# tomer-erez/Psychoacoustic-adverserial-attacks

Hardware: AMD Instinct MI355X
Metric: pgd_steps_per_sec (higher is better)
Workload: dtype bf16x3 (split-bf16 hi+lo, three MFMA passes, f32 accumulate: fp32-parity); 1 GPU; untargeted PGD, norm_type snr snr_db 40, Wav2Vec2-base (rule-generated weights), 32x10s 16 kHz clips per GPU, 150-token labels; global_batch=32, per_gpu_batch=32, samples_per_clip=160000, parallelism=dp1, hip_graph=True, hip_graph_replayed_steps=80

## Files before the change

### psychoacoustic-adverserial-attacks_amd/csrc/gemm.hip

```cpp
#include <algorithm>
#include <vector>

#include "gemm_dev.h"

namespace paa {

template <int ROWS, bool IS_A>
__device__ __forceinline__ void load_kc(const paa_gemm_desc& d, const float* __restrict__ base, int64_t ld, int r0,
                                        int k0, int rlim, float4 (&v)[ROWS / 32]) {
    const int tid = threadIdx.x;
    const int k = k0 + ((tid & 7) << 2);
    int64_t koff = k;
    int js = 0, kc = k;
    if (IS_A && d.a_kseg > 0) {
        js = k / d.a_kseg;
        kc = k - js * d.a_kseg;
        koff = (int64_t)js * d.a_kseg_stride + kc;
    }
#pragma unroll
    for (int i = 0; i < ROWS / 32; ++i) {
        const int r = r0 + (tid >> 3) + 32 * i;
        float4 x = make_float4(0.f, 0.f, 0.f, 0.f);
        bool ok = (r < rlim) && (k < d.K);
        const float* p;
        if (IS_A && d.a_window) {
            const int tr = r + js - d.a_pad;
            ok = ok && (tr >= 0) && (tr < d.a_rows_valid);
            p = base + (int64_t)tr * ld + kc;
        } else {
            p = base + (int64_t)r * ld + koff;
        }
        if (ok) {
// ... 518 lines not shown
    const int total = g.tiles_m * g.tiles_n * g.d.batch;
    const int blocks = resident > 0 ? std::min(total, resident) : total;
    hipLaunchKernelGGL((k_gemm_bf<BM, BN, PREC, WM, VEC, SEG, SWZ>), dim3(blocks), dim3(WM * 128), 0, st, g);
}

void launch_ring_cfg(int cfg, const GemmArgs& g, hipStream_t st);
void launch_ring2_cfg(int cfg, const GemmArgs& g, hipStream_t st);
int ring_tile_rows(int cfg);
int ring_tile_cols(int cfg);
bool ring_cfg_ok(int cfg, const paa_gemm_desc& d, bool forced = false);

static int g_ring_mode = 0;
struct GemmEnv { bool init = false, no_sq = false, no_r2 = false, kgroup = true, no_bil = false; };
static GemmEnv g_env;
static void gemm_env_refresh() {
#ifdef PAA_EXPERIMENTS
    auto on = [](const char* name, char v) { const char* e = getenv(name); return e && e[0] == v; };
    g_env.no_sq = on("PAA_NO_SQ", '1');
    g_env.no_r2 = on("PAA_NO_R2", '1');
    g_env.kgroup = !on("PAA_K_GROUP", '0');
    g_env.no_bil = on("PAA_NO_BIL", '1');
#endif
    g_env.init = true;
}
bool gemm_env_no_bil() {
    if (!g_env.init) gemm_env_refresh();
    return g_env.no_bil;
}
bool gemm_env_kgroup() {
    if (!g_env.init) gemm_env_refresh();
    return g_env.kgroup;
}

static int g_last_kind = EPK_GENERIC;
static int classify_epilogue(const paa_gemm_desc& d) {
#ifdef PAA_EXPERIMENTS
    { const char* e = getenv("PAA_NO_EPIK"); if (e && e[0] == '1') return EPK_GENERIC; }
#endif
    if (d.alpha != 1.f || d.accumulate || d.aux_bf16 || !d.precision) return EPK_GENERIC;
    const bool il = d.Cb_il && !d.Cb && !d.Cb_lo, planar = d.Cb && d.Cb_lo && !d.Cb_il, no_planes = !d.Cb && !d.Cb_lo && !d.Cb_il;
    const bool mask = d.row_period > 0;
    switch (d.act) {
        case PAA_ACT_GELU:
            return (d.C_pre && d.aux_gate && il && !d.C && !d.aux && !d.residual && !d.res_ln_stats) ? EPK_GELU_FWD : EPK_GENERIC;
        case PAA_ACT_GELU_GRAD:
            if (!(d.aux && d.aux_gate && (il || planar) && !d.bias && !d.C && !d.C_pre && !d.residual && !d.res_ln_stats && !mask)) return EPK_GENERIC;
#ifdef PAA_EXPERIMENTS
            { const char* e = getenv("PAA_EPIK_AHEAD"); if (e && e[0] == '2') return EPK_GELU_GRAD_LA2; if (e && e[0] == '4') return EPK_GELU_GRAD_LA4;
              if (e && e[0] == '1') return EPK_GELU_GRAD_LA1; }
#endif
            return EPK_GELU_GRAD;
        case PAA_ACT_NONE:
            if (d.C_pre || d.aux || d.aux_gate || mask) return EPK_GENERIC;
            if (d.C && no_planes && d.residual) {
                if (d.res_ln_stats) return d.bias ? EPK_RESID_LN : EPK_GENERIC;
                return d.bias ? EPK_GENERIC : EPK_RESID;
            }
            if (!d.C && planar && !d.residual && !d.res_ln_stats) return EPK_PLANES;
            return EPK_GENERIC;
        default: return EPK_GENERIC;
    }
}

template <int BN, int PREC>
static void launch_gemm(const GemmArgs& g, dim3 grid, hipStream_t st) {
    const bool akc = g.d.a_kcontig != 0, bkc = g.d.b_kcontig != 0;
    if (akc && bkc) hipLaunchKernelGGL((k_gemm<BN, PREC, true, true>), grid, dim3(G_NT), 0, st, g);
    else if (akc && !bkc) hipLaunchKernelGGL((k_gemm<BN, PREC, true, false>), grid, dim3(G_NT), 0, st, g);
    else if (!akc && bkc) hipLaunchKernelGGL((k_gemm<BN, PREC, false, true>), grid, dim3(G_NT), 0, st, g);
    else hipLaunchKernelGGL((k_gemm<BN, PREC, false, false>), grid, dim3(G_NT), 0, st, g);
}

struct GemmProf {
    bool on = false;
    std::vector<hipEvent_t> ev;
    std::vector<double> flops, bytes;
    std::vector<int> variant;
    size_t n = 0, cap = 0;
};
static GemmProf g_prof;

paa_status gemm(const paa_gemm_desc& d, hipStream_t st) {
    if ((!d.A && !d.A_il) || !d.B || (!d.C && !d.Cb && !d.Cb_il)) PAA_FAIL(PAA_ERR_ARG, "gemm: null operand");
    if (d.A_il) {
        if (!d.precision || !d.operand_bf16 || d.a_kseg > 0 || d.a_window || (d.lda & 31) || (d.K & 31) || (d.a_s1 & 31) || (d.a_s2 & 31) || ((uintptr_t)d.A_il & 15))
            PAA_FAIL(PAA_ERR_ARG, "gemm: A_il needs split precision, plain K-contiguous bf16 rows and lda / K / batch strides that are multiples of 32");
    }
    if (d.Cb_il) {
        if (!d.precision || d.Cb || d.Cb_lo || (d.ldc & 31) || (d.c_s1 & 31) || (d.c_s2 & 31) || ((uintptr_t)d.Cb_il & 15))
            PAA_FAIL(PAA_ERR_ARG, "gemm: Cb_il needs split precision, no Cb / Cb_lo, and ldc / batch strides that are multiples of 32");
    }
    if (d.accumulate && !d.C) PAA_FAIL(PAA_ERR_ARG, "gemm: accumulate needs the f32 result");
    if (d.Cb_lo && !d.Cb) PAA_FAIL(PAA_ERR_ARG, "gemm: Cb_lo without Cb");
    if (d.M <= 0 || d.N <= 0 || d.K <= 0 || d.batch <= 0 || d.batch2 <= 0) PAA_FAIL(PAA_ERR_SIZE, "gemm: bad dims %d %d %d", d.M, d.N, d.K);
    const int al = d.operand_bf16 ? 7 : 3;
    if ((d.lda & al) || (d.ldb & al) || (!d.A_il && ((uintptr_t)d.A & 15)) || ((uintptr_t)d.B & 15))
        PAA_FAIL(PAA_ERR_ARG, "gemm: operands must be 16-byte aligned with leading dimensions that are multiples of %d", al + 1);
    if ((d.a_s1 & al) || (d.a_s2 & al) || (d.b_s1 & al) || (d.b_s2 & al)) PAA_FAIL(PAA_ERR_ARG, "gemm: batch strides must be multiples of %d", al + 1);
    if (d.a_kseg > 0 && ((d.a_kseg & al) || (d.a_kseg_stride & al) || !d.a_kcontig)) PAA_FAIL(PAA_ERR_ARG, "gemm: bad K segmentation");
    if (d.operand_bf16) {
        if (!d.a_kcontig || !d.b_kcontig || (d.K & 7)) PAA_FAIL(PAA_ERR_ARG, "gemm: bf16 operands must be K-contiguous with K %% 8 == 0 (K=%d)", d.K);
        if (d.precision && ((!d.A_il && (!d.A_lo || ((uintptr_t)d.A_lo & 15))) || !d.B_lo || ((uintptr_t)d.B_lo & 15)))
            PAA_FAIL(PAA_ERR_ARG, "gemm: split precision needs aligned lo planes");
    }
    if (d.a_window && d.a_kseg <= 0) PAA_FAIL(PAA_ERR_ARG, "gemm: a_window needs a_kseg");
    if (d.act == PAA_ACT_GELU_GRAD && !d.aux) PAA_FAIL(PAA_ERR_ARG, "gemm: GELU_GRAD needs aux");
    if (d.res_ln_stats && (!d.residual || !d.res_ln_g || !d.res_ln_b || d.batch != 1 || d.act == PAA_ACT_GELU_GRAD ||
                           ((uintptr_t)d.res_ln_stats & 7) || ((uintptr_t)d.res_ln_g & 15) || ((uintptr_t)d.res_ln_b & 15)))
        PAA_FAIL(PAA_ERR_ARG, "gemm: res_ln_stats needs a residual, gain and bias (16-byte aligned), batch 1 and no GELU_GRAD");
    GemmArgs g;
    g.d = d;
    g.kind = EPK_GENERIC;
    const bool narrow = d.N <= 64;
    const int bn = narrow ? 64 : 128;
    auto al16 = [](const void* p) { return ((uintptr_t)p & 15) == 0; };
    const bool vec = d.operand_bf16 && !narrow && (d.N & 7) == 0 && (d.ldc & 7) == 0 && (d.c_s1 & 7) == 0 && (d.c_s2 & 7) == 0 &&
                     al16(d.C) && al16(d.C_pre) && al16(d.Cb) && al16(d.Cb_lo) && al16(d.Cb_il) &&
                     (!d.aux || (al16(d.aux) && (d.ld_aux & (d.aux_bf16 ? 7 : 3)) == 0 && (d.aux_s1 & 7) == 0 && (d.aux_s2 & 7) == 0)) &&
                     (!d.residual || (al16(d.residual) && (d.ld_res & 3) == 0 && (d.res_s1 & 3) == 0 && (d.res_s2 & 3) == 0)) &&
                     (!d.bias || (al16(d.bias) && (d.bias_s2 & 3) == 0)) &&
                     !(d.act == PAA_ACT_GELU_GRAD && d.residual) &&
                     63 * d.lda < (1ll << 30) && 63 * d.ldb < (1ll << 30) && (int64_t)d.M * d.ldc < (1ll << 30) && (int64_t)d.M * std::max(d.ld_aux, d.ld_res) < (1ll << 30);
    const bool tall = vec && d.a_kseg <= 0 && (d.K & 63) == 0 && d.M >= 2048;
    bool bm192 = false;
    if (tall && !d.precision) {
        static const int per_cu = std::max(1, blocks_per_cu(k_gemm_bf<256, 128, 0, 2, true, false>, 256));
        const int slots = per_cu * device_cus();
        const int64_t tn = cdiv(d.N, 128);
        const int64_t t256 = (int64_t)cdiv(d.M, 256) * tn * d.batch, t192 = (int64_t)cdiv(d.M, 192) * tn * d.batch;
        const double c256 = (double)((t256 + slots - 1) / slots) * 256.0, c192 = (double)((t192 + slots - 1) / slots) * 192.0 * 1.05;
        bm192 = c192 < c256;
    }
    int ring = 0;
    const bool forced2 = g_ring_mode >= 20 && vec && d.a_kseg <= 0 && ring_cfg_ok(g_ring_mode, d, true);
    if ((tall || forced2) && g_ring_mode != 1 && d.N >= 128) {
        const int64_t t256 = (int64_t)cdiv(d.M, 256) * cdiv(d.N, 256) * d.batch, t128 = (int64_t)cdiv(d.M, 256) * cdiv(d.N, 128) * d.batch;
        if (!g_env.init) gemm_env_refresh();
        const bool no_sq = g_env.no_sq;
        if (g_ring_mode >= 2) ring = g_ring_mode;
        else if (d.precision) {
            const int64_t slots = device_cus();
            const int64_t r256 = (t128 + slots - 1) / slots;
            const int64_t t192 = (int64_t)cdiv(d.M, 192) * cdiv(d.N, 128) * d.batch;
            const int64_t r192 = (t192 + 2 * slots - 1) / (2 * slots);
            const int64_t rsq = (t256 + slots - 1) / slots;
// ... 61 lines not shown
        const size_t lds = 2 * (size_t)npl * ((size_t)(128 * mi + taps - 1) * (d.a_kseg + 8) + 64 * (size_t)(4 * d.a_kseg + 8));
        if (lds <= 150 * 1024) {
            dim3 wgrid(cdiv(d.M, 128 * mi), d.batch);
#define PAA_WIN(P, KS_, MI_, WV_)                                                                                            \
            {                                                                                                                \
                static bool attr = false;                                                                                    \
                if (!attr) { PAA_HIP(hipFuncSetAttribute(reinterpret_cast<const void*>(&k_gemm_win<P, KS_, MI_, WV_>), hipFuncAttributeMaxDynamicSharedMemorySize, 152 * 1024)); attr = true; } \
                hipLaunchKernelGGL((k_gemm_win<P, KS_, MI_, WV_>), wgrid, dim3(WV_ * 64), lds, st, g, taps);                 \
            }
            if (prof) { g_prof.variant[g_prof.n] = 40 + (d.precision ? 4 : 0); }
            if (d.a_kseg == 48) {
                if (mi == 2) { if (d.precision) PAA_WIN(1, 48, 1, 8) else PAA_WIN(0, 48, 2, 4) }
                else { if (d.precision) PAA_WIN(1, 48, 1, 4) else PAA_WIN(0, 48, 1, 4) }
            }
            else { if (d.precision) PAA_WIN(1, 64, 1, 4) else PAA_WIN(0, 64, 1, 4) }
#undef PAA_WIN
            if (prof) { (void)hipEventRecord(g_prof.ev[2 * g_prof.n + 1], st); ++g_prof.n; }
            PAA_LAUNCH_CHECK();
            return PAA_OK;
        }
    }
    if (ring) {
        if (prof) g_prof.variant[g_prof.n] = (ring_bm == 192 ? (ring_bn == 128 ? 60 : 52) : (ring_bn == 256 ? 56 : 48)) + (d.precision ? 1 : 0);
#ifdef PAA_EXPERIMENTS
        if (ring == 13) launch_bf<192, 128, 1, 2, true, false, true>(g, st);
        else
#endif
        if (ring >= 20) {
            g.kind = g_last_kind = classify_epilogue(d);
            int taken = EPK_SHIPPED;
#ifdef PAA_EXPERIMENTS
            { const char* e = getenv("PAA_EPIK_MASK"); const int mask = e ? atoi(e) : 0; if (mask > 0) taken = mask; }
#endif
            if (!((taken >> g.kind) & 1)) g.kind = EPK_GENERIC;
            launch_ring2_cfg(ring, g, st);
        }
        else launch_ring_cfg(ring, g, st);
    } else if (d.operand_bf16) {
        const bool seg = d.a_kseg > 0 || (d.K & 63);
        if (narrow) {
            if (seg) { if (d.precision) launch_bf<128, 64, 1, 2, false, true>(g, st); else launch_bf<128, 64, 0, 2, false, true>(g, st); }
            else { if (d.precision) launch_bf<128, 64, 1, 2, false, false>(g, st); else launch_bf<128, 64, 0, 2, false, false>(g, st); }
        }
        else if (seg && vec && !d.precision) launch_bf<128, 128, 0, 2, true, true>(g, st);
        else if (seg) { if (d.precision) launch_bf<128, 128, 1, 2, false, true>(g, st); else launch_bf<128, 128, 0, 2, false, true>(g, st); }
        else if (tall) {
            if (d.precision) launch_bf<256, 128, 1, 4, true, false>(g, st);
            else if (bm192) launch_bf<192, 128, 0, 2, true, false>(g, st);
            else launch_bf<256, 128, 0, 2, true, false>(g, st);
        }
        else if (vec) { if (d.precision) launch_bf<128, 128, 1, 2, true, false>(g, st); else launch_bf<128, 128, 0, 2, true, false>(g, st); }
        else { if (d.precision) launch_bf<128, 128, 1, 2, false, false>(g, st); else launch_bf<128, 128, 0, 2, false, false>(g, st); }
    } else if (narrow) { if (d.precision) launch_gemm<64, 1>(g, grid, st); else launch_gemm<64, 0>(g, grid, st); }
    else { if (d.precision) launch_gemm<128, 1>(g, grid, st); else launch_gemm<128, 0>(g, grid, st); }
    if (prof) { (void)hipEventRecord(g_prof.ev[2 * g_prof.n + 1], st); ++g_prof.n; }
    PAA_LAUNCH_CHECK();
    return PAA_OK;
}

}

extern "C" paa_status paa_prof_enable(int max_launches) {
    using namespace paa;
    for (hipEvent_t e : g_prof.ev) (void)hipEventDestroy(e);
    g_prof.ev.clear(); g_prof.n = 0; g_prof.cap = 0; g_prof.on = false;
    if (max_launches <= 0) return PAA_OK;
    g_prof.ev.resize(2 * (size_t)max_launches);
    for (auto& e : g_prof.ev) PAA_HIP(hipEventCreate(&e));
    g_prof.flops.assign(max_launches, 0.0);
    g_prof.bytes.assign(max_launches, 0.0);
    g_prof.variant.assign(max_launches, 0);
    g_prof.cap = max_launches; g_prof.on = true;
    return PAA_OK;
}

extern "C" paa_status paa_prof_read(double* out256) {
    using namespace paa;
    if (!out256) PAA_FAIL(PAA_ERR_ARG, "paa_prof_read: null");
    for (int i = 0; i < 256; ++i) out256[i] = 0.0;
    if (g_prof.n == 0) return PAA_OK;
    PAA_HIP(hipEventSynchronize(g_prof.ev[2 * g_prof.n - 1]));
    for (size_t i = 0; i < g_prof.n; ++i) {
        float ms = 0.f;
        PAA_HIP(hipEventElapsedTime(&ms, g_prof.ev[2 * i], g_prof.ev[2 * i + 1]));
        const int v = g_prof.variant[i];
        out256[4 * v] += 1.0; out256[4 * v + 1] += ms; out256[4 * v + 2] += g_prof.flops[i]; out256[4 * v + 3] += g_prof.bytes[i];
    }
    g_prof.n = 0;
    return PAA_OK;
}

extern "C" paa_status paa_prof_pause(int paused) {
    paa::g_prof.on = !paused && paa::g_prof.cap > 0;
    return PAA_OK;
}

#ifdef PAA_EXPERIMENTS
extern "C" int paa_debug_last_epilogue_kind() { return paa::g_last_kind; }
#endif

extern "C" void paa_gemm_config(int ring_mode) { paa::g_ring_mode = ring_mode; paa::gemm_env_refresh(); }

extern "C" paa_status paa_gemm(const struct paa_gemm_desc* d, void* stream) {
    if (!d) { paa::set_error("paa_gemm: null descriptor"); return PAA_ERR_ARG; }
    return paa::gemm(*d, (hipStream_t)stream);
}
```

### psychoacoustic-adverserial-attacks_amd/csrc/gemm_dev.h

```cpp
#pragma once
#include "gemm.h"
#include "paa_common.h"

namespace paa {

typedef short bf16x8 __attribute__((ext_vector_type(8)));
typedef float f32x16 __attribute__((ext_vector_type(16)));

constexpr int G_BM = 128, G_BK = 32, G_LD = 40 , G_NT = 256;


struct GemmArgs {
    paa_gemm_desc d;
    int tiles_m, tiles_n;
    int kind;
};

enum { EPK_GENERIC = 0, EPK_GELU_FWD = 1, EPK_GELU_GRAD = 2, EPK_RESID = 3, EPK_RESID_LN = 4, EPK_PLANES = 5,
       EPK_GELU_GRAD_LA2 = 6, EPK_GELU_GRAD_LA4 = 7, EPK_GELU_GRAD_LA1 = 8, EPK_COUNT = 9 };
constexpr int EPK_SHIPPED = (1 << EPK_GELU_FWD) | (1 << EPK_GELU_GRAD) | (1 << EPK_PLANES);
enum { EPI_NO = 0, EPI_YES = 1, EPI_RT = 2 };
template <int S>
__device__ __forceinline__ bool epi_on(bool rt) {
    if constexpr (S == EPI_RT) return rt;
    else return S == EPI_YES;
}
struct EpiGeneric {
    static constexpr int ACT = -1, BIAS = EPI_RT, C = EPI_RT, CPRE = EPI_RT, X16 = EPI_RT, GATE = EPI_RT, CIL = EPI_RT, CB = EPI_RT, CBLO = EPI_RT,
                         RES = EPI_RT, RLN = EPI_RT, PERIOD = EPI_RT, ACCUM = EPI_RT;
    static constexpr bool ALPHA1 = false;
    static constexpr int AHEAD = 1;
    static constexpr bool SETTLE_EARLY = false;
};
struct EpiGeluFwd {
    static constexpr int ACT = PAA_ACT_GELU, BIAS = EPI_RT, C = EPI_NO, CPRE = EPI_YES, X16 = EPI_NO, GATE = EPI_YES, CIL = EPI_YES, CB = EPI_NO, CBLO = EPI_NO,
                         RES = EPI_NO, RLN = EPI_NO, PERIOD = EPI_RT, ACCUM = EPI_NO;
    static constexpr bool ALPHA1 = true;
    static constexpr int AHEAD = 1;
    static constexpr bool SETTLE_EARLY = false;
};
struct EpiGeluGrad {
    static constexpr int ACT = PAA_ACT_GELU_GRAD, BIAS = EPI_NO, C = EPI_NO, CPRE = EPI_NO, X16 = EPI_NO, GATE = EPI_YES, CIL = EPI_RT, CB = EPI_YES, CBLO = EPI_YES,
                         RES = EPI_NO, RLN = EPI_NO, PERIOD = EPI_NO, ACCUM = EPI_NO;
    static constexpr bool ALPHA1 = true;
    static constexpr int AHEAD = 1;
    static constexpr bool SETTLE_EARLY = true;
};
template <int AH>
struct EpiGeluGradAhead : EpiGeluGrad {
    static constexpr int AHEAD = AH;
    static constexpr bool SETTLE_EARLY = false;
};
struct EpiResid {
    static constexpr int ACT = PAA_ACT_NONE, BIAS = EPI_NO, C = EPI_YES, CPRE = EPI_NO, X16 = EPI_NO, GATE = EPI_NO, CIL = EPI_NO, CB = EPI_NO, CBLO = EPI_NO,
                         RES = EPI_YES, RLN = EPI_NO, PERIOD = EPI_NO, ACCUM = EPI_NO;
    static constexpr bool ALPHA1 = true;
    static constexpr int AHEAD = 1;
    static constexpr bool SETTLE_EARLY = false;
};
struct EpiResidLn {
    static constexpr int ACT = PAA_ACT_NONE, BIAS = EPI_YES, C = EPI_YES, CPRE = EPI_NO, X16 = EPI_NO, GATE = EPI_NO, CIL = EPI_NO, CB = EPI_NO, CBLO = EPI_NO,
                         RES = EPI_YES, RLN = EPI_YES, PERIOD = EPI_NO, ACCUM = EPI_NO;
    static constexpr bool ALPHA1 = true;
    static constexpr int AHEAD = 1;
    static constexpr bool SETTLE_EARLY = false;
};
struct EpiPlanes {
    static constexpr int ACT = PAA_ACT_NONE, BIAS = EPI_RT, C = EPI_NO, CPRE = EPI_NO, X16 = EPI_NO, GATE = EPI_NO, CIL = EPI_NO, CB = EPI_YES, CBLO = EPI_YES,
                         RES = EPI_NO, RLN = EPI_NO, PERIOD = EPI_NO, ACCUM = EPI_NO;
    static constexpr bool ALPHA1 = true;
    static constexpr int AHEAD = 1;
    static constexpr bool SETTLE_EARLY = false;
};

template <typename K>
inline int blocks_per_cu(K kernel, int threads) {
    int per = 0;
    if (hipOccupancyMaxActiveBlocksPerMultiprocessor(&per, kernel, threads, 0) != hipSuccess) return 0;
    return per;
}

template <int NJ, int MI>
__device__ __forceinline__ void epilogue(const paa_gemm_desc& d, f32x16 (&acc)[MI][NJ], int mw, int nw, int z1, int z2) {
    const int64_t coff = z1 * d.c_s1 + z2 * d.c_s2 + (int64_t)mw * d.ldc + nw;
    float* __restrict__ C = d.C ? d.C + coff : nullptr;
    const bool x16 = d.aux_bf16 != 0;
    float* __restrict__ Cp = (d.C_pre && !x16) ? d.C_pre + coff : nullptr;
    unsigned short* __restrict__ Cp16 = (d.C_pre && x16) ? reinterpret_cast<unsigned short*>(d.C_pre) + coff : nullptr;
    unsigned short* __restrict__ Cb = d.Cb ? reinterpret_cast<unsigned short*>(d.Cb) + coff : nullptr;
    unsigned short* __restrict__ Cbl = d.Cb_lo ? reinterpret_cast<unsigned short*>(d.Cb_lo) + coff : nullptr;
    unsigned short* __restrict__ Cil = d.Cb_il ? reinterpret_cast<unsigned short*>(d.Cb_il) + 2 * (z1 * d.c_s1 + z2 * d.c_s2) : nullptr;
    const int64_t xoff = z1 * d.aux_s1 + z2 * d.aux_s2 + (int64_t)mw * d.ld_aux + nw;
    const float* __restrict__ aux = (d.aux && !x16) ? d.aux + xoff : nullptr;
    const unsigned short* __restrict__ aux16 = (d.aux && x16) ? reinterpret_cast<const unsigned short*>(d.aux) + xoff : nullptr;
    const float* __restrict__ res = d.residual ? d.residual + z1 * d.res_s1 + z2 * d.res_s2 + (int64_t)mw * d.ld_res + nw : nullptr;
    const float* __restrict__ bias = d.bias ? d.bias + z2 * d.bias_s2 + nw : nullptr;
    const int ldc = (int)d.ldc, ld_aux = (int)d.ld_aux, ld_res = (int)d.ld_res;
    const int period = d.row_period;
    const int mrem0 = period > 0 ? mw % period : 0;
    const int act = d.act;
    const float alpha = d.alpha;
#pragma unroll
    for (int i = 0; i < MI; ++i) {
        const int64_t ro = (int64_t)(i * 32) * ldc;
        float* __restrict__ Ci = C ? C + ro : nullptr;
// ... 57 lines not shown
                }
                if (Cil) {
                    const int n = nw + dn;
                    const int64_t o = (int64_t)(mw + i * 32 + dm) * (2 * d.ldc) + ((n >> 5) << 6) + (n & 31);
                    const unsigned short h = bf16_bits(v);
                    Cil[o] = h;
                    Cil[o + 32] = bf16_bits(v - bf16_to_f32(h));
                }
            }
        }
    }
}

__device__ __forceinline__ float dpp_quad_xor1(float v) {
    return __int_as_float(__builtin_amdgcn_mov_dpp(__float_as_int(v), 0xB1, 0xF, 0xF, true));
}
__device__ __forceinline__ float dpp_quad_xor2(float v) {
    return __int_as_float(__builtin_amdgcn_mov_dpp(__float_as_int(v), 0x4E, 0xF, 0xF, true));
}
__device__ __forceinline__ void quad_transpose(float& x0, float& x1, float& x2, float& x3, bool o1, bool o2) {
    float s = dpp_quad_xor1(o1 ? x0 : x1);
    float t = dpp_quad_xor1(o1 ? x2 : x3);
    if (o1) { x0 = s; x2 = t; } else { x1 = s; x3 = t; }
    s = dpp_quad_xor2(o2 ? x0 : x2);
    t = dpp_quad_xor2(o2 ? x1 : x3);
    if (o2) { x0 = s; x1 = t; } else { x2 = s; x3 = t; }
}

__device__ __forceinline__ float mul_unfused(float a, float b) {
#pragma clang fp contract(off)
    return a * b;
}

__device__ __forceinline__ void epi_landed(const uint4& v) { asm volatile("" ::"v"(v.x), "v"(v.y), "v"(v.z), "v"(v.w)); }
template <int N>
__device__ __forceinline__ void epi_landed(const float (&v)[N]) {
#pragma unroll
    for (int k = 0; k < N; ++k) asm volatile("" ::"v"(v[k]));
}

template <int MI, bool FAST, typename T = EpiGeneric>
__device__ __forceinline__ void epilogue_vec(const paa_gemm_desc& d, f32x16 (&acc)[MI][2], int m0w, int n0w, int z1, int z2, int lane) {
    const int lr = lane & 31, lh = lane >> 5, qa = lr >> 2, qb = lr & 3;
    const bool o1 = qb & 1, o2 = qb & 2;
    const int col = n0w + 8 * qa;
    const int row0 = m0w + 4 * lh + qb;
    const bool col_ok = col < d.N;
    const int act = T::ACT < 0 ? d.act : T::ACT;
    const bool gg = act == PAA_ACT_GELU_GRAD;
    const int64_t cbase = z1 * d.c_s1 + z2 * d.c_s2;
    float* __restrict__ C = epi_on<T::C>(d.C != nullptr) ? d.C + cbase : nullptr;
    const bool has_c = T::C == EPI_RT ? C != nullptr : T::C == EPI_YES;
    const bool x16 = epi_on<T::X16>(d.aux_bf16 != 0);
    const bool gate = epi_on<T::GATE>(d.aux_gate != 0);
    float* __restrict__ Cp = (epi_on<T::CPRE>(d.C_pre != nullptr) && !x16) ? d.C_pre + cbase : nullptr;
    unsigned short* __restrict__ Cp16 = (epi_on<T::CPRE>(d.C_pre != nullptr) && x16) ? reinterpret_cast<unsigned short*>(d.C_pre) + cbase : nullptr;
    constexpr bool PRE_RT = T::CPRE == EPI_RT || T::X16 == EPI_RT;
    const bool has_cp = PRE_RT ? Cp != nullptr : (T::CPRE == EPI_YES && T::X16 == EPI_NO);
    const bool has_cp16 = PRE_RT ? Cp16 != nullptr : (T::CPRE == EPI_YES && T::X16 == EPI_YES);
    unsigned short* __restrict__ Cb = epi_on<T::CB>(d.Cb != nullptr) ? reinterpret_cast<unsigned short*>(d.Cb) + cbase : nullptr;
    unsigned short* __restrict__ Cbl = epi_on<T::CBLO>(d.Cb_lo != nullptr) ? reinterpret_cast<unsigned short*>(d.Cb_lo) + cbase : nullptr;
    const bool cil = epi_on<T::CIL>(d.Cb_il != nullptr);
    if (cil) { Cb = reinterpret_cast<unsigned short*>(d.Cb_il) + 2 * cbase; Cbl = Cb + 32; }
    const bool has_cb = (T::CIL == EPI_YES || T::CB == EPI_YES) ? true : (T::CIL == EPI_NO && T::CB == EPI_NO) ? false : Cb != nullptr;
    const bool has_cbl = (T::CIL == EPI_YES || T::CBLO == EPI_YES) ? true : (T::CIL == EPI_NO && T::CBLO == EPI_NO) ? false : Cbl != nullptr;
    const bool ex16 = gg && x16;
    const float* __restrict__ ex = gg ? (ex16 ? nullptr : d.aux + z1 * d.aux_s1 + z2 * d.aux_s2)
                                      : (epi_on<T::RES>(d.residual != nullptr) ? d.residual + z1 * d.res_s1 + z2 * d.res_s2 : nullptr);
    const unsigned short* __restrict__ exh = ex16 ? reinterpret_cast<const unsigned short*>(d.aux) + z1 * d.aux_s1 + z2 * d.aux_s2 : nullptr;
    constexpr bool EX_RT = T::ACT < 0 || T::X16 == EPI_RT || T::RES == EPI_RT;
    const bool has_ex = EX_RT ? ex != nullptr : (gg ? !ex16 : T::RES == EPI_YES);
    const bool has_exh = EX_RT ? exh != nullptr : ex16;
    const unsigned ldc = (unsigned)d.ldc, ldx = (unsigned)(gg ? d.ld_aux : d.ld_res);
    const unsigned co = (unsigned)row0 * ldc + (unsigned)col;
    const unsigned cob = cil ? (unsigned)row0 * 2u * ldc + (((unsigned)col >> 5) << 6) + ((unsigned)col & 31u) : co;
    const unsigned ldcb = cil ? 2u * ldc : ldc;
    float bv[8];
#pragma unroll
    for (int k = 0; k < 8; ++k) bv[k] = 0.f;
    if (epi_on<T::BIAS>(d.bias != nullptr) && col_ok) {
        const float* bp = d.bias + z2 * d.bias_s2;
        const float4 b0 = *reinterpret_cast<const float4*>(bp + (unsigned)col);
        const float4 b1 = *reinterpret_cast<const float4*>(bp + (unsigned)col + 4u);
        bv[0] = b0.x; bv[1] = b0.y; bv[2] = b0.z; bv[3] = b0.w; bv[4] = b1.x; bv[5] = b1.y; bv[6] = b1.z; bv[7] = b1.w;
    }
    const bool rln = epi_on<T::RLN>(d.res_ln_stats != nullptr) && !gg && has_ex;
    constexpr bool RLN_HELD = MI < 4;
    float lg[8], lb[8];
#pragma unroll
    for (int k = 0; k < 8; ++k) { lg[k] = 1.f; lb[k] = 0.f; }
    if (RLN_HELD && rln && col_ok) {
        const float4 g0 = *reinterpret_cast<const float4*>(d.res_ln_g + (unsigned)col), g1 = *reinterpret_cast<const float4*>(d.res_ln_g + (unsigned)col + 4u);
        const float4 b0 = *reinterpret_cast<const float4*>(d.res_ln_b + (unsigned)col), b1 = *reinterpret_cast<const float4*>(d.res_ln_b + (unsigned)col + 4u);
        lg[0] = g0.x; lg[1] = g0.y; lg[2] = g0.z; lg[3] = g0.w; lg[4] = g1.x; lg[5] = g1.y; lg[6] = g1.z; lg[7] = g1.w;
        lb[0] = b0.x; lb[1] = b0.y; lb[2] = b0.z; lb[3] = b0.w; lb[4] = b1.x; lb[5] = b1.y; lb[6] = b1.z; lb[7] = b1.w;
    }
    const int period = T::PERIOD == EPI_NO ? 0 : d.row_period;
    const int mrem0 = period > 0 ? row0 % period : 0;
    const float alpha = T::ALPHA1 ? 1.f : d.alpha;
    const bool accum = epi_on<T::ACCUM>(d.accumulate != 0);
    constexpr int NG = 4 * MI;
    constexpr int AH = T::AHEAD < NG ? T::AHEAD : NG - 1, NX = AH + 1;
    uint4 xv[NX][2];
    constexpr bool RS_AHEAD = T::RLN == EPI_YES;
    float rsv[NX][2];
    constexpr bool EARLY = T::SETTLE_EARLY && AH == 1 && T::ACT == PAA_ACT_GELU_GRAD && T::X16 != EPI_RT && T::C == EPI_NO && T::CPRE == EPI_NO;
    constexpr bool EX_ANY = EX_RT || T::ACT == PAA_ACT_GELU_GRAD || T::RES == EPI_YES;
#pragma unroll
    for (int u = 0; u < NX; ++u) { xv[u][0] = make_uint4(0u, 0u, 0u, 0u); xv[u][1] = xv[u][0]; rsv[u][0] = 0.f; rsv[u][1] = 1.f; }
    auto fetch = [&](int grp, uint4 (&v2)[2], float (&r2)[2]) {
        const unsigned rowc = (unsigned)min(row0 + (grp >> 2) * 32 + (grp & 3) * 8, d.M - 1);
        if (RS_AHEAD && rln) {
            const float2 st = *reinterpret_cast<const float2*>(d.res_ln_stats + 2 * (size_t)rowc);
            r2[0] = st.x; r2[1] = st.y;
        }
        const unsigned o = rowc * ldx + (col_ok ? (unsigned)col : 0u);
        if (has_ex) {
            v2[0] = *reinterpret_cast<const uint4*>(ex + o);
            v2[1] = *reinterpret_cast<const uint4*>(ex + o + 4u);
        } else if (has_exh) {
            v2[0] = *reinterpret_cast<const uint4*>(exh + o);
        }
    };
#pragma unroll
    for (int a = 0; a < AH; ++a) fetch(a, xv[a], rsv[a]);
#pragma unroll
    for (int grp = 0; grp < NG; ++grp) {
        const int i = grp >> 2, gq = grp & 3, u = grp % NX;
        if (grp + AH < NG) fetch(grp + AH, xv[(grp + AH) % NX], rsv[(grp + AH) % NX]);
        if (grp == 0) {
            if constexpr (T::BIAS != EPI_NO) epi_landed(bv);
            if constexpr (RLN_HELD && T::RLN != EPI_NO) { epi_landed(lg); epi_landed(lb); }
        }
        if constexpr (EX_ANY) { epi_landed(xv[u][0]); epi_landed(xv[u][1]); }
        if constexpr (RS_AHEAD) epi_landed(rsv[u]);
        const int dm = i * 32 + gq * 8;
        const bool live = col_ok && row0 + dm < d.M;
        bool dead = false;
        if (period > 0) {
            int rem = mrem0 + dm;
            if (rem >= period) rem = (period >= 256) ? rem - period : rem % period;
            dead = rem >= d.row_valid;
        }
        const unsigned ci = co + (unsigned)dm * ldc;
        float2 rst = make_float2(rsv[u][0], rsv[u][1]);
        if (!RS_AHEAD && rln && live) rst = *reinterpret_cast<const float2*>(d.res_ln_stats + 2 * (size_t)(row0 + dm));
        unsigned hp[4], lp[4], pp[4];
#pragma unroll
        for (int j = 0; j < 2; ++j) {
            float x[4] = {acc[i][j][4 * gq], acc[i][j][4 * gq + 1], acc[i][j][4 * gq + 2], acc[i][j][4 * gq + 3]};
            quad_transpose(x[0], x[1], x[2], x[3], o1, o2);
            float e4[4];
            if (ex16) {
                const unsigned w0 = j ? xv[u][0].z : xv[u][0].x, w1 = j ? xv[u][0].w : xv[u][0].y;
                e4[0] = __uint_as_float(w0 << 16); e4[1] = __uint_as_float(w0 & 0xFFFF0000u);
                e4[2] = __uint_as_float(w1 << 16); e4[3] = __uint_as_float(w1 & 0xFFFF0000u);
            } else {
                e4[0] = __uint_as_float(xv[u][j].x); e4[1] = __uint_as_float(xv[u][j].y);
                e4[2] = __uint_as_float(xv[u][j].z); e4[3] = __uint_as_float(xv[u][j].w);
            }
            if (rln) {
                if constexpr (RLN_HELD) {
#pragma unroll
                    for (int k = 0; k < 4; ++k) e4[k] = (e4[k] - rst.x) * rst.y * lg[4 * j + k] + lb[4 * j + k];
                } else {
                    float4 g4 = make_float4(1.f, 1.f, 1.f, 1.f), b4 = make_float4(0.f, 0.f, 0.f, 0.f);
                    if (col_ok) {
                        g4 = *reinterpret_cast<const float4*>(d.res_ln_g + (unsigned)col + 4u * j);
                        b4 = *reinterpret_cast<const float4*>(d.res_ln_b + (unsigned)col + 4u * j);
                    }
                    e4[0] = (e4[0] - rst.x) * rst.y * g4.x + b4.x; e4[1] = (e4[1] - rst.x) * rst.y * g4.y + b4.y;
                    e4[2] = (e4[2] - rst.x) * rst.y * g4.z + b4.z; e4[3] = (e4[3] - rst.x) * rst.y * g4.w + b4.w;
                }
            }
#pragma unroll
            for (int k = 0; k < 4; ++k) x[k] = x[k] * alpha + bv[4 * j + k];
            if (act == PAA_ACT_GELU) {
                float kp[4];
                if (FAST) {
#pragma unroll
                    for (int k = 0; k < 4; k += 2) {
                        f32x2 dg;
                        const f32x2 gv = gelu_both_fast2(f32x2{x[k], x[k + 1]}, dg);
                        kp[k] = gate ? dg.x : x[k]; kp[k + 1] = gate ? dg.y : x[k + 1];
                        x[k] = gv.x; x[k + 1] = gv.y;
                    }
                } else {
#pragma unroll
                    for (int k = 0; k < 4; ++k) {
                        kp[k] = gate ? gelu_grad_f(x[k]) : x[k];
                        x[k] = gelu_f(x[k]);
                    }
                }
                if (has_cp && live) *reinterpret_cast<float4*>(Cp + ci + 4u * j) = dead ? make_float4(0.f, 0.f, 0.f, 0.f) : make_float4(kp[0], kp[1], kp[2], kp[3]);
                if (has_cp16) {
                    pp[2 * j] = dead ? 0u : bf16_pack2(kp[0], kp[1]);
                    pp[2 * j + 1] = dead ? 0u : bf16_pack2(kp[2], kp[3]);
                }
                if (has_ex) {
#pragma unroll
                    for (int k = 0; k < 4; ++k) x[k] += e4[k];
                }
            } else if (gg) {
#pragma unroll
                for (int k = 0; k < 4; ++k) x[k] = mul_unfused(x[k], gate ? e4[k] : (FAST ? gelu_grad_fast(e4[k]) : gelu_grad_f(e4[k])));
            } else if (has_ex) {
#pragma unroll
                for (int k = 0; k < 4; ++k) x[k] += e4[k];
            }
            if (dead) {
#pragma unroll
                for (int k = 0; k < 4; ++k) x[k] = 0.f;
            }
            if (has_c && live) {
                if (accum) {
                    const float4 c0 = *reinterpret_cast<const float4*>(C + ci + 4u * j);
                    x[0] += c0.x; x[1] += c0.y; x[2] += c0.z; x[3] += c0.w;
                }
                *reinterpret_cast<float4*>(C + ci + 4u * j) = make_float4(x[0], x[1], x[2], x[3]);
            }
            if (has_cb) {
                const unsigned h01 = bf16_pack2(x[0], x[1]), h23 = bf16_pack2(x[2], x[3]);
                hp[2 * j] = h01; hp[2 * j + 1] = h23;
                if (has_cbl) {
                    lp[2 * j] = bf16_pack2(x[0] - __uint_as_float(h01 << 16), x[1] - __uint_as_float(h01 & 0xFFFF0000u));
                    lp[2 * j + 1] = bf16_pack2(x[2] - __uint_as_float(h23 << 16), x[3] - __uint_as_float(h23 & 0xFFFF0000u));
                }
            }
            __builtin_amdgcn_sched_barrier(0);
        }
        if constexpr (EARLY) {
            if (grp + 1 < NG) { epi_landed(xv[(grp + 1) % NX][0]); epi_landed(xv[(grp + 1) % NX][1]); }
        }
        if (has_cp16 && live && act == PAA_ACT_GELU) *reinterpret_cast<uint4*>(Cp16 + ci) = make_uint4(pp[0], pp[1], pp[2], pp[3]);
        if (has_cb && live) {
            const unsigned cb = cob + (unsigned)dm * ldcb;
            *reinterpret_cast<uint4*>(Cb + cb) = make_uint4(hp[0], hp[1], hp[2], hp[3]);
            if (has_cbl) *reinterpret_cast<uint4*>(Cbl + cb) = make_uint4(lp[0], lp[1], lp[2], lp[3]);
        }
    }
}

}
```

### psychoacoustic-adverserial-attacks_amd/csrc/gemm_ring2.hip

```cpp
#include <stdlib.h>

#include <algorithm>

#include "gemm_dev.h"

namespace paa {

bool gemm_env_no_bil();

namespace {

#if defined(PAA_R2_DEFER) && !defined(PAA_EXPERIMENTS)
#error "PAA_R2_DEFER is a diagnostic build: add -DPAA_EXPERIMENTS"
#endif
#ifndef PAA_R2_DEFER
#define PAA_R2_DEFER 1
#endif
#if (defined(PAA_R2_A_AUX) || defined(PAA_R2_B_AUX)) && !defined(PAA_EXPERIMENTS)
#error "PAA_R2_A_AUX / PAA_R2_B_AUX are diagnostic builds: add -DPAA_EXPERIMENTS"
#endif
#ifndef PAA_R2_A_AUX
#define PAA_R2_A_AUX 0
#endif
#ifndef PAA_R2_PRIO_BALANCE
// ... 311 lines not shown
                            for (int j = 0; j < NJ; ++j) { bh[j] = bhn[j]; bl[j] = bln[j]; }
                        }
                    }
                }
            if (!DEFER || last) {
                if (ahead) wait_vmcnt2<GA>(); else wait_vmcnt2<0>();
                __builtin_amdgcn_sched_barrier(0);
                __builtin_amdgcn_s_barrier();
                __builtin_amdgcn_sched_barrier(0);
            }
        }
#ifdef PAA_R2_STAMP
        const long long st_t1 = R2_NOW();
#endif
        epilogue_vec<MI, true, EPI>(d, acc, cur.m0 + wr * (BM / WR), cur.n0 + wc * (BN / WC), cur.z1, cur.z2, lane);
#ifdef PAA_R2_STAMP
        if (blockIdx.x == 0 && lane == 0 && st_tile < 16) {
            long long* o = g_r2_stamp + (wave * 16 + st_tile) * 6;
            o[0] = nk; o[1] = st_t1 - st_t0; o[2] = st_vm; o[3] = st_bar; o[4] = R2_NOW() - st_t1; o[5] = st_t0;
        }
        ++st_tile;
#endif
    }
}

template <int BM, int BN, int BK, int PREC, int WR, int WC, bool BIL, bool AIL, typename EPI = EpiGeneric>
void launch_ring2_il(const GemmArgs& g, hipStream_t st) {
    static const int per_cu = blocks_per_cu(k_gemm_ring2<BM, BN, BK, PREC, WR, WC, BIL, AIL, EPI>, WR * WC * 64);
    const int resident = per_cu * device_cus();
    const int total = g.tiles_m * g.tiles_n * g.d.batch;
    const int blocks = resident > 0 ? std::min(total, resident) : total;
    hipLaunchKernelGGL((k_gemm_ring2<BM, BN, BK, PREC, WR, WC, BIL, AIL, EPI>), dim3(blocks), dim3(WR * WC * 64), 0, st, g);
}
template <int BM, int BN, int BK, int WR, int WC, bool AIL>
void launch_ring2_kind(const GemmArgs& g, hipStream_t st) {
    switch (g.kind) {
        case EPK_GELU_FWD: launch_ring2_il<BM, BN, BK, 1, WR, WC, true, AIL, EpiGeluFwd>(g, st); return;
        case EPK_GELU_GRAD: launch_ring2_il<BM, BN, BK, 1, WR, WC, true, AIL, EpiGeluGrad>(g, st); return;
#ifdef PAA_EXPERIMENTS
        case EPK_GELU_GRAD_LA2: launch_ring2_il<BM, BN, BK, 1, WR, WC, true, AIL, EpiGeluGradAhead<2>>(g, st); return;
        case EPK_GELU_GRAD_LA4: launch_ring2_il<BM, BN, BK, 1, WR, WC, true, AIL, EpiGeluGradAhead<4>>(g, st); return;
        case EPK_GELU_GRAD_LA1: launch_ring2_il<BM, BN, BK, 1, WR, WC, true, AIL, EpiGeluGradAhead<1>>(g, st); return;
#endif
        default: break;
    }
    if constexpr (BM == 192) {
        switch (g.kind) {
            case EPK_PLANES: launch_ring2_il<BM, BN, BK, 1, WR, WC, true, AIL, EpiPlanes>(g, st); return;
#ifdef PAA_EXPERIMENTS
            case EPK_RESID: launch_ring2_il<BM, BN, BK, 1, WR, WC, true, AIL, EpiResid>(g, st); return;
            case EPK_RESID_LN: launch_ring2_il<BM, BN, BK, 1, WR, WC, true, AIL, EpiResidLn>(g, st); return;
#endif
            default: break;
        }
    }
    launch_ring2_il<BM, BN, BK, 1, WR, WC, true, AIL>(g, st);
}
template <int BM, int BN, int BK, int PREC, int WR, int WC>
void launch_ring2(const GemmArgs& g, hipStream_t st) {
    if constexpr (PREC == 1) {
        const bool bil = g.d.B_il && g.d.b_s1 == 0 && g.d.b_s2 == 0 && !gemm_env_no_bil();
        if (g.d.A_il) {
            if (bil) launch_ring2_kind<BM, BN, BK, WR, WC, true>(g, st);
            else launch_ring2_il<BM, BN, BK, PREC, WR, WC, false, true>(g, st);
            return;
        }
        if (bil) { launch_ring2_kind<BM, BN, BK, WR, WC, false>(g, st); return; }
    }
    launch_ring2_il<BM, BN, BK, PREC, WR, WC, false, false>(g, st);
}

}

#ifdef PAA_R2_STAMP
}
extern "C" int paa_debug_r2_stamps(long long* host) {
    if (hipDeviceSynchronize() != hipSuccess) return 1;
    if (hipMemcpyFromSymbol(host, HIP_SYMBOL(paa::g_r2_stamp), sizeof(long long) * 8 * 16 * 6) != hipSuccess) return 1;
    static long long zeros[8 * 16 * 6];
    return hipMemcpyToSymbol(HIP_SYMBOL(paa::g_r2_stamp), zeros, sizeof(zeros)) == hipSuccess ? 0 : 1;
}
namespace paa {
#endif

void launch_ring2_cfg(int cfg, const GemmArgs& g, hipStream_t st) {
// ... 11 lines not shown
```

Measured before the change: 29.26 steps/s (one step = PGD step on 32 x 10 s clips; counted over all ranks).

## Ship residual and residual-LN fused epilogues with buffer-resource stores

Enables the specialised residual and residual+LayerNorm epilogue kernels in the shipped mask, where before only experimental builds reached them. The GELU-grad, residual and residual-LN epilogues now write through raw buffer stores with a wave-uniform base, and out-of-range rows are dropped by the hardware bounds check instead of by per-lane branches. Lookahead depth becomes a template parameter chosen per kind. The LN step is computed with contraction off to keep bit-parity, and large ldc falls back to the generic epilogue. The aim is fewer instructions and branches in the epilogue, at the cost of more template instantiations and a possible numerical difference from the generic path.

```diff
diff --git a/psychoacoustic-adverserial-attacks_amd/csrc/gemm.hip b/psychoacoustic-adverserial-attacks_amd/csrc/gemm.hip
--- a/psychoacoustic-adverserial-attacks_amd/csrc/gemm.hip
+++ b/psychoacoustic-adverserial-attacks_amd/csrc/gemm.hip
@@ -1,3 +1,5 @@
+#include <stdio.h>
+
 #include <algorithm>
 #include <vector>
 
@@ -582,7 +584,21 @@
     return g_env.kgroup;
 }
 
-static int g_last_kind = EPK_GENERIC;
+static int g_last_kind = EPK_GENERIC, g_last_ahead = 0;
+static int epilogue_ahead(int kind) {
+    const int slot = kind == EPK_GELU_GRAD ? 0 : kind == EPK_RESID ? 1 : kind == EPK_RESID_LN ? 2 : -1;
+    if (slot < 0) return 0;
+    const int shipped[3] = {EPI_AHEAD_GELU_GRAD, EPI_AHEAD_RESID, EPI_AHEAD_RESID_LN};
+#ifdef PAA_EXPERIMENTS
+    if (const char* e = getenv("PAA_EPIK_AHEAD")) {
+        int v[3] = {0, 0, 0};
+        const int n = sscanf(e, "%d,%d,%d", &v[0], &v[1], &v[2]);
+        const int a = n == 1 ? v[0] : n == 3 ? v[slot] : 0;
+        if (a >= 1 && a <= EPI_AHEAD_MAX) return a;
+    }
+#endif
+    return shipped[slot];
+}
 static int classify_epilogue(const paa_gemm_desc& d) {
 #ifdef PAA_EXPERIMENTS
     { const char* e = getenv("PAA_NO_EPIK"); if (e && e[0] == '1') return EPK_GENERIC; }
@@ -595,10 +611,6 @@
             return (d.C_pre && d.aux_gate && il && !d.C && !d.aux && !d.residual && !d.res_ln_stats) ? EPK_GELU_FWD : EPK_GENERIC;
         case PAA_ACT_GELU_GRAD:
             if (!(d.aux && d.aux_gate && (il || planar) && !d.bias && !d.C && !d.C_pre && !d.residual && !d.res_ln_stats && !mask)) return EPK_GENERIC;
-#ifdef PAA_EXPERIMENTS
-            { const char* e = getenv("PAA_EPIK_AHEAD"); if (e && e[0] == '2') return EPK_GELU_GRAD_LA2; if (e && e[0] == '4') return EPK_GELU_GRAD_LA4;
-              if (e && e[0] == '1') return EPK_GELU_GRAD_LA1; }
-#endif
             return EPK_GELU_GRAD;
         case PAA_ACT_NONE:
             if (d.C_pre || d.aux || d.aux_gate || mask) return EPK_GENERIC;
@@ -661,6 +673,7 @@
     GemmArgs g;
     g.d = d;
     g.kind = EPK_GENERIC;
+    g.ahead = 0;
     const bool narrow = d.N <= 64;
     const int bn = narrow ? 64 : 128;
     auto al16 = [](const void* p) { return ((uintptr_t)p & 15) == 0; };
@@ -788,7 +801,8 @@
 #ifdef PAA_EXPERIMENTS
             { const char* e = getenv("PAA_EPIK_MASK"); const int mask = e ? atoi(e) : 0; if (mask > 0) taken = mask; }
 #endif
-            if (!((taken >> g.kind) & 1)) g.kind = EPK_GENERIC;
+            if (!((taken >> g.kind) & 1) || d.ldc >= (1 << 21)) g.kind = EPK_GENERIC;
+            g.ahead = g_last_ahead = epilogue_ahead(g.kind);
             launch_ring2_cfg(ring, g, st);
         }
         else launch_ring_cfg(ring, g, st);
@@ -853,6 +867,7 @@
 
 #ifdef PAA_EXPERIMENTS
 extern "C" int paa_debug_last_epilogue_kind() { return paa::g_last_kind; }
+extern "C" int paa_debug_last_epilogue_ahead() { return paa::g_last_ahead; }
 #endif
 
 extern "C" void paa_gemm_config(int ring_mode) { paa::g_ring_mode = ring_mode; paa::gemm_env_refresh(); }
diff --git a/psychoacoustic-adverserial-attacks_amd/csrc/gemm_dev.h b/psychoacoustic-adverserial-attacks_amd/csrc/gemm_dev.h
--- a/psychoacoustic-adverserial-attacks_amd/csrc/gemm_dev.h
+++ b/psychoacoustic-adverserial-attacks_amd/csrc/gemm_dev.h
@@ -14,11 +14,13 @@
     paa_gemm_desc d;
     int tiles_m, tiles_n;
     int kind;
-};
-
-enum { EPK_GENERIC = 0, EPK_GELU_FWD = 1, EPK_GELU_GRAD = 2, EPK_RESID = 3, EPK_RESID_LN = 4, EPK_PLANES = 5,
-       EPK_GELU_GRAD_LA2 = 6, EPK_GELU_GRAD_LA4 = 7, EPK_GELU_GRAD_LA1 = 8, EPK_COUNT = 9 };
-constexpr int EPK_SHIPPED = (1 << EPK_GELU_FWD) | (1 << EPK_GELU_GRAD) | (1 << EPK_PLANES);
+    int ahead;
+};
+
+enum { EPK_GENERIC = 0, EPK_GELU_FWD = 1, EPK_GELU_GRAD = 2, EPK_RESID = 3, EPK_RESID_LN = 4, EPK_PLANES = 5, EPK_COUNT = 6 };
+constexpr int EPK_SHIPPED = (1 << EPK_GELU_FWD) | (1 << EPK_GELU_GRAD) | (1 << EPK_PLANES) | (1 << EPK_RESID) | (1 << EPK_RESID_LN);
+constexpr int EPI_AHEAD_MAX = 4;
+constexpr int EPI_AHEAD_GELU_GRAD = 1, EPI_AHEAD_RESID = 1, EPI_AHEAD_RESID_LN = 1;
 enum { EPI_NO = 0, EPI_YES = 1, EPI_RT = 2 };
 template <int S>
 __device__ __forceinline__ bool epi_on(bool rt) {
@@ -31,6 +33,7 @@
     static constexpr bool ALPHA1 = false;
     static constexpr int AHEAD = 1;
     static constexpr bool SETTLE_EARLY = false;
+    static constexpr bool BUF_STORES = false;
 };
 struct EpiGeluFwd {
     static constexpr int ACT = PAA_ACT_GELU, BIAS = EPI_RT, C = EPI_NO, CPRE = EPI_YES, X16 = EPI_NO, GATE = EPI_YES, CIL = EPI_YES, CB = EPI_NO, CBLO = EPI_NO,
@@ -38,32 +41,34 @@
     static constexpr bool ALPHA1 = true;
     static constexpr int AHEAD = 1;
     static constexpr bool SETTLE_EARLY = false;
-};
-struct EpiGeluGrad {
+    static constexpr bool BUF_STORES = false;
+};
+template <int AH>
+struct EpiGeluGradA {
     static constexpr int ACT = PAA_ACT_GELU_GRAD, BIAS = EPI_NO, C = EPI_NO, CPRE = EPI_NO, X16 = EPI_NO, GATE = EPI_YES, CIL = EPI_RT, CB = EPI_YES, CBLO = EPI_YES,
                          RES = EPI_NO, RLN = EPI_NO, PERIOD = EPI_NO, ACCUM = EPI_NO;
     static constexpr bool ALPHA1 = true;
-    static constexpr int AHEAD = 1;
+    static constexpr int AHEAD = AH;
     static constexpr bool SETTLE_EARLY = true;
+    static constexpr bool BUF_STORES = true;
 };
 template <int AH>
-struct EpiGeluGradAhead : EpiGeluGrad {
-    static constexpr int AHEAD = AH;
-    static constexpr bool SETTLE_EARLY = false;
-};
-struct EpiResid {
+struct EpiResidA {
     static constexpr int ACT = PAA_ACT_NONE, BIAS = EPI_NO, C = EPI_YES, CPRE = EPI_NO, X16 = EPI_NO, GATE = EPI_NO, CIL = EPI_NO, CB = EPI_NO, CBLO = EPI_NO,
                          RES = EPI_YES, RLN = EPI_NO, PERIOD = EPI_NO, ACCUM = EPI_NO;
     static constexpr bool ALPHA1 = true;
-    static constexpr int AHEAD = 1;
+    static constexpr int AHEAD = AH;
     static constexpr bool SETTLE_EARLY = false;
-};
-struct EpiResidLn {
+    static constexpr bool BUF_STORES = true;
+};
+template <int AH>
+struct EpiResidLnA {
     static constexpr int ACT = PAA_ACT_NONE, BIAS = EPI_YES, C = EPI_YES, CPRE = EPI_NO, X16 = EPI_NO, GATE = EPI_NO, CIL = EPI_NO, CB = EPI_NO, CBLO = EPI_NO,
                          RES = EPI_YES, RLN = EPI_YES, PERIOD = EPI_NO, ACCUM = EPI_NO;
     static constexpr bool ALPHA1 = true;
-    static constexpr int AHEAD = 1;
+    static constexpr int AHEAD = AH;
     static constexpr bool SETTLE_EARLY = false;
+    static constexpr bool BUF_STORES = true;
 };
 struct EpiPlanes {
     static constexpr int ACT = PAA_ACT_NONE, BIAS = EPI_RT, C = EPI_NO, CPRE = EPI_NO, X16 = EPI_NO, GATE = EPI_NO, CIL = EPI_NO, CB = EPI_YES, CBLO = EPI_YES,
@@ -71,6 +76,7 @@
     static constexpr bool ALPHA1 = true;
     static constexpr int AHEAD = 1;
     static constexpr bool SETTLE_EARLY = false;
+    static constexpr bool BUF_STORES = false;
 };
 
 template <typename K>
@@ -194,11 +200,36 @@
     return a * b;
 }
 
+__device__ __forceinline__ float ln_residual(float x, float mean, float rstd, float gain, float bias) {
+#pragma clang fp contract(off)
+    return __builtin_fmaf((x - mean) * rstd, gain, bias);
+}
+
 __device__ __forceinline__ void epi_landed(const uint4& v) { asm volatile("" ::"v"(v.x), "v"(v.y), "v"(v.z), "v"(v.w)); }
 template <int N>
 __device__ __forceinline__ void epi_landed(const float (&v)[N]) {
 #pragma unroll
     for (int k = 0; k < N; ++k) asm volatile("" ::"v"(v[k]));
+}
+
+struct EpiBuf { unsigned lo, hi, bytes; };
+constexpr unsigned EPI_DROP = 0x80000000u;
+__device__ __forceinline__ EpiBuf epi_buf(const void* base, long long bytes) {
+    EpiBuf b{0u, 0u, 0u};
+#if defined(__HIP_DEVICE_COMPILE__)
+    const unsigned long long p = (unsigned long long)base;
+    b.lo = (unsigned)__builtin_amdgcn_readfirstlane((int)(unsigned)p);
+    b.hi = (unsigned)__builtin_amdgcn_readfirstlane((int)(p >> 32));
+    b.bytes = (unsigned)__builtin_amdgcn_readfirstlane((int)(bytes < 0 ? 0 : bytes > (long long)EPI_DROP ? (long long)EPI_DROP : bytes));
+#endif
+    return b;
+}
+__device__ __forceinline__ void epi_store16(const EpiBuf& b, unsigned off, unsigned x, unsigned y, unsigned z, unsigned w) {
+#if defined(__HIP_DEVICE_COMPILE__)
+    typedef unsigned u32x4 __attribute__((ext_vector_type(4)));
+    const unsigned long long p = ((unsigned long long)b.hi << 32) | b.lo;
+    __builtin_amdgcn_raw_buffer_store_b128(u32x4{x, y, z, w}, __builtin_amdgcn_make_buffer_rsrc((void*)p, 0, (int)b.bytes, 0x00020000), (int)off, 0, 0);
+#endif
 }
 
 template <int MI, bool FAST, typename T = EpiGeneric>
@@ -237,6 +268,20 @@
     const unsigned co = (unsigned)row0 * ldc + (unsigned)col;
     const unsigned cob = cil ? (unsigned)row0 * 2u * ldc + (((unsigned)col >> 5) << 6) + ((unsigned)col & 31u) : co;
     const unsigned ldcb = cil ? 2u * ldc : ldc;
+    constexpr bool BUF = T::BUF_STORES;
+    static_assert(!BUF || (T::C != EPI_RT && T::CB != EPI_RT && T::CBLO != EPI_RT && T::CPRE == EPI_NO && T::ACCUM == EPI_NO && T::PERIOD == EPI_NO),
+                  "buffer stores: a folded kind whose stores are the f32 result or the planes, nothing read back");
+    EpiBuf bufC{0u, 0u, 0u}, bufB = bufC, bufL = bufC;
+    unsigned ol = 0u, olb = 0u;
+    if constexpr (BUF) {
+        const long long wrows = min(MI * 32, d.M - m0w);
+        const unsigned r0 = (unsigned)(4 * lh + qb);
+        ol = (r0 * ldc + (unsigned)col) * 4u;
+        olb = (cil ? r0 * 2u * ldc + (((unsigned)col >> 5) << 6) + ((unsigned)col & 31u) : r0 * ldc + (unsigned)col) * 2u;
+        if (has_c) bufC = epi_buf(C + (int64_t)m0w * ldc, wrows * ldc * 4);
+        if (has_cb) bufB = epi_buf(Cb + (int64_t)m0w * ldcb, wrows * ldcb * 2);
+        if (has_cbl) bufL = epi_buf(Cbl + (int64_t)m0w * ldcb, wrows * ldcb * 2 - (cil ? 64 : 0));
+    }
     float bv[8];
 #pragma unroll
     for (int k = 0; k < 8; ++k) bv[k] = 0.f;
@@ -266,7 +311,7 @@
     uint4 xv[NX][2];
     constexpr bool RS_AHEAD = T::RLN == EPI_YES;
     float rsv[NX][2];
-    constexpr bool EARLY = T::SETTLE_EARLY && AH == 1 && T::ACT == PAA_ACT_GELU_GRAD && T::X16 != EPI_RT && T::C == EPI_NO && T::CPRE == EPI_NO;
+    constexpr bool EARLY = T::SETTLE_EARLY && T::ACT == PAA_ACT_GELU_GRAD && T::X16 != EPI_RT && T::C == EPI_NO && T::CPRE == EPI_NO;
     constexpr bool EX_ANY = EX_RT || T::ACT == PAA_ACT_GELU_GRAD || T::RES == EPI_YES;
 #pragma unroll
     for (int u = 0; u < NX; ++u) { xv[u][0] = make_uint4(0u, 0u, 0u, 0u); xv[u][1] = xv[u][0]; rsv[u][0] = 0.f; rsv[u][1] = 1.f; }
@@ -324,15 +369,15 @@
             if (rln) {
                 if constexpr (RLN_HELD) {
 #pragma unroll
-                    for (int k = 0; k < 4; ++k) e4[k] = (e4[k] - rst.x) * rst.y * lg[4 * j + k] + lb[4 * j + k];
+                    for (int k = 0; k < 4; ++k) e4[k] = ln_residual(e4[k], rst.x, rst.y, lg[4 * j + k], lb[4 * j + k]);
                 } else {
                     float4 g4 = make_float4(1.f, 1.f, 1.f, 1.f), b4 = make_float4(0.f, 0.f, 0.f, 0.f);
                     if (col_ok) {
                         g4 = *reinterpret_cast<const float4*>(d.res_ln_g + (unsigned)col + 4u * j);
                         b4 = *reinterpret_cast<const float4*>(d.res_ln_b + (unsigned)col + 4u * j);
                     }
-                    e4[0] = (e4[0] - rst.x) * rst.y * g4.x + b4.x; e4[1] = (e4[1] - rst.x) * rst.y * g4.y + b4.y;
-                    e4[2] = (e4[2] - rst.x) * rst.y * g4.z + b4.z; e4[3] = (e4[3] - rst.x) * rst.y * g4.w + b4.w;
+                    e4[0] = ln_residual(e4[0], rst.x, rst.y, g4.x, b4.x); e4[1] = ln_residual(e4[1], rst.x, rst.y, g4.y, b4.y);
+                    e4[2] = ln_residual(e4[2], rst.x, rst.y, g4.z, b4.z); e4[3] = ln_residual(e4[3], rst.x, rst.y, g4.w, b4.w);
                 }
             }
 #pragma unroll
@@ -374,7 +419,9 @@
 #pragma unroll
                 for (int k = 0; k < 4; ++k) x[k] = 0.f;
             }
-            if (has_c && live) {
+            if constexpr (BUF) {
+                if (has_c) epi_store16(bufC, live ? ol + ((unsigned)dm * ldc + 4u * j) * 4u : EPI_DROP, __float_as_uint(x[0]), __float_as_uint(x[1]), __float_as_uint(x[2]), __float_as_uint(x[3]));
+            } else if (has_c && live) {
                 if (accum) {
                     const float4 c0 = *reinterpret_cast<const float4*>(C + ci + 4u * j);
                     x[0] += c0.x; x[1] += c0.y; x[2] += c0.z; x[3] += c0.w;
@@ -395,7 +442,13 @@
             if (grp + 1 < NG) { epi_landed(xv[(grp + 1) % NX][0]); epi_landed(xv[(grp + 1) % NX][1]); }
         }
         if (has_cp16 && live && act == PAA_ACT_GELU) *reinterpret_cast<uint4*>(Cp16 + ci) = make_uint4(pp[0], pp[1], pp[2], pp[3]);
-        if (has_cb && live) {
+        if constexpr (BUF) {
+            if (has_cb) {
+                const unsigned ob = live ? olb + (unsigned)dm * ldcb * 2u : EPI_DROP;
+                epi_store16(bufB, ob, hp[0], hp[1], hp[2], hp[3]);
+                if (has_cbl) epi_store16(bufL, ob, lp[0], lp[1], lp[2], lp[3]);
+            }
+        } else if (has_cb && live) {
             const unsigned cb = cob + (unsigned)dm * ldcb;
             *reinterpret_cast<uint4*>(Cb + cb) = make_uint4(hp[0], hp[1], hp[2], hp[3]);
             if (has_cbl) *reinterpret_cast<uint4*>(Cbl + cb) = make_uint4(lp[0], lp[1], lp[2], lp[3]);
diff --git a/psychoacoustic-adverserial-attacks_amd/csrc/gemm_ring2.hip b/psychoacoustic-adverserial-attacks_amd/csrc/gemm_ring2.hip
--- a/psychoacoustic-adverserial-attacks_amd/csrc/gemm_ring2.hip
+++ b/psychoacoustic-adverserial-attacks_amd/csrc/gemm_ring2.hip
@@ -367,25 +367,32 @@
     const int blocks = resident > 0 ? std::min(total, resident) : total;
     hipLaunchKernelGGL((k_gemm_ring2<BM, BN, BK, PREC, WR, WC, BIL, AIL, EPI>), dim3(blocks), dim3(WR * WC * 64), 0, st, g);
 }
+template <int BM, int BN, int BK, int WR, int WC, bool AIL, template <int> class KIND, int SHIP>
+void launch_ring2_depth(const GemmArgs& g, hipStream_t st) {
+#ifdef PAA_EXPERIMENTS
+    static_assert(EPI_AHEAD_MAX == 4, "one case per depth");
+    switch (g.ahead) {
+        case 1: launch_ring2_il<BM, BN, BK, 1, WR, WC, true, AIL, KIND<1>>(g, st); return;
+        case 2: launch_ring2_il<BM, BN, BK, 1, WR, WC, true, AIL, KIND<2>>(g, st); return;
+        case 3: launch_ring2_il<BM, BN, BK, 1, WR, WC, true, AIL, KIND<3>>(g, st); return;
+        case 4: launch_ring2_il<BM, BN, BK, 1, WR, WC, true, AIL, KIND<4>>(g, st); return;
+        default: break;
+    }
+#endif
+    launch_ring2_il<BM, BN, BK, 1, WR, WC, true, AIL, KIND<SHIP>>(g, st);
+}
 template <int BM, int BN, int BK, int WR, int WC, bool AIL>
 void launch_ring2_kind(const GemmArgs& g, hipStream_t st) {
     switch (g.kind) {
         case EPK_GELU_FWD: launch_ring2_il<BM, BN, BK, 1, WR, WC, true, AIL, EpiGeluFwd>(g, st); return;
-        case EPK_GELU_GRAD: launch_ring2_il<BM, BN, BK, 1, WR, WC, true, AIL, EpiGeluGrad>(g, st); return;
-#ifdef PAA_EXPERIMENTS
-        case EPK_GELU_GRAD_LA2: launch_ring2_il<BM, BN, BK, 1, WR, WC, true, AIL, EpiGeluGradAhead<2>>(g, st); return;
-        case EPK_GELU_GRAD_LA4: launch_ring2_il<BM, BN, BK, 1, WR, WC, true, AIL, EpiGeluGradAhead<4>>(g, st); return;
-        case EPK_GELU_GRAD_LA1: launch_ring2_il<BM, BN, BK, 1, WR, WC, true, AIL, EpiGeluGradAhead<1>>(g, st); return;
-#endif
+        case EPK_GELU_GRAD: launch_ring2_depth<BM, BN, BK, WR, WC, AIL, EpiGeluGradA, EPI_AHEAD_GELU_GRAD>(g, st); return;
         default: break;
     }
     if constexpr (BM == 192) {
         switch (g.kind) {
             case EPK_PLANES: launch_ring2_il<BM, BN, BK, 1, WR, WC, true, AIL, EpiPlanes>(g, st); return;
-#ifdef PAA_EXPERIMENTS
-            case EPK_RESID: launch_ring2_il<BM, BN, BK, 1, WR, WC, true, AIL, EpiResid>(g, st); return;
-            case EPK_RESID_LN: launch_ring2_il<BM, BN, BK, 1, WR, WC, true, AIL, EpiResidLn>(g, st); return;
-#endif
+            case EPK_RESID: launch_ring2_depth<BM, BN, BK, WR, WC, AIL, EpiResidA, EPI_AHEAD_RESID>(g, st); return;
+            case EPK_RESID_LN: launch_ring2_depth<BM, BN, BK, WR, WC, AIL, EpiResidLnA, EPI_AHEAD_RESID_LN>(g, st); return;
             default: break;
         }
     }
```

Result: no change. 29.45 steps/s (one step = PGD step on 32 x 10 s clips; counted over all ranks) (median of 6 runs) (+0.7%).
